# Emieeel/auto_oo

Hardware: NVIDIA B200
Metric: oo_energy_gradient_hessian_evals_per_sec (higher is better)
Workload: dtype f64

## Files before the change

auto_oo_b200/csrc/classes.cu:

```cuda
#include "common.cuh"

namespace oo {

int dgemm_tn(const double *At, const double *B, double *C, int64_t M, int64_t N, int64_t K,
             int64_t lda, int64_t ldb, int64_t ldc, int batch, int64_t strideA, int64_t strideB,
             int64_t strideC, cudaStream_t stream);
int dgemm_tn_swap02(const double *At, const double *B, double *C, double *C2, int d0, int d1, int d2,
                    int64_t N, int64_t K, int64_t lda, int64_t ldb, int64_t ldc, int batch, int64_t strideA,
                    int64_t strideB, int64_t strideC, cudaStream_t stream);
int dgemm_tn_pair_unpack(const double *At, const double *B, double *C, double *C2, int d0, int dorb, int dP,
                         int64_t N, int64_t K, int64_t lda, int64_t ldb, int64_t ldc, int batch,
                         int64_t strideA, int64_t strideB, int64_t strideC, int64_t strideC2,
                         cudaStream_t stream);

int dgemm_tn_class_pack(const double *At, const double *B, double *P, int tri_rows, int nclass, int dorb,
                        int64_t nrows2, int64_t npair_ld, int64_t K, int64_t lda, int64_t ldb, int batch,
                        int64_t strideA, int64_t strideB, int64_t strideP, cudaStream_t stream, int64_t r2_offset = 0);

int dgemm_tn_q1_packed8(const double *A8, int64_t a8_ld, int pq_lo, int pq_cnt, const double *B, double *C,
                        double *C2, int dorb, int dP, int64_t N, int64_t K, int64_t ldb, int64_t ldc, int batch,
                        int64_t strideA8, int64_t strideB, int64_t strideC, int64_t strideC2, cudaStream_t stream,
                        bool direct_epilogue);
bool dgemm_tn_tri_supported(int nclass);
int dgemm_tn_tri_class_pack(const double *At, const double *B, double *P, int tri_rows, int nclass, int dorb,
                            int64_t ngroups, int64_t npair_ld, int64_t K, int64_t lda, int64_t ldb, int batch,
                            int64_t strideA, int64_t strideB, int64_t strideP, cudaStream_t stream,
                            int64_t group_offset = 0, int64_t group_ld = 0, int halves = 1);

int dgemm_tn_class_expand(const double *At, const double *B, double *Out, int transpose_mirror, int nclass, int dorb,
                          int64_t npair_ld, int64_t K, int64_t lda, int64_t ldb, int64_t ld_out, int batch,
                          int64_t strideA, int64_t strideB, int64_t strideOut, cudaStream_t stream,
                          bool direct_epilogue = false);
int dgemm_tn_direct(const double *At, const double *B, double *C, int64_t M, int64_t N, int64_t K,
                    int64_t lda, int64_t ldb, int64_t ldc, int batch, int64_t strideA, int64_t strideB,
                    int64_t strideC, cudaStream_t stream);

namespace {

__global__ void __launch_bounds__(256) transpose_kernel(const double *__restrict__ src,
                                                        double *__restrict__ dst, int64_t rows,
                                                        int64_t cols) {
    __shared__ double tile[32][33];
    const int64_t c0 = (int64_t)blockIdx.x * 32, r0 = (int64_t)blockIdx.y * 32;
    const int tx = threadIdx.x & 31, ty = threadIdx.x >> 5;
#pragma unroll
    for (int j = ty; j < 32; j += 8) {
        const int64_t r = r0 + j, c = c0 + tx;
        if (r < rows && c < cols) tile[j][tx] = src[r * cols + c];
    }
    __syncthreads();
#pragma unroll
    for (int j = ty; j < 32; j += 8) {
        const int64_t c = c0 + j, r = r0 + tx;
        if (r < rows && c < cols) dst[c * rows + r] = tile[tx][j];
    }
}

}

int transpose(const double *src, double *dst, int64_t rows, int64_t cols, cudaStream_t stream) {
// ... 289 lines not shown
    if (!run(0)) {
    } else if (flags & OO_FLAG_CLASS_ERI_8FOLD) {
        if (slab) {
            OO_CUDA_CHECK(cudaMemsetAsync(T1t, 0, (size_t)batch * sT1t * sizeof(double), stream));
            OO_CUDA_CHECK(cudaMemsetAsync(P0, 0, (size_t)batch * sXp * sizeof(double), stream));
        }
        if (npairs) {
            concat_class_columns_kernel<<<dim3((unsigned)ld, (unsigned)npairs), 64, 0, stream>>>(C, strideC, ld, nIp, X);
            OO_LAUNCH_CHECK();
            if ((rc = dgemm_tn_q1_packed8(gpk, ldp, 0, (int)ldp, X, T1, T1t, ld, (int)ldp, 2 * nIp, ld, 2 * nIp, 2 * nIp,
                                          npairs, 0, (int64_t)ld * 2 * nIp, 2 * sT1, 2 * sT1t, stream, direct)))
                return rc;
        }
        if (nsingle &&
            (rc = dgemm_tn_q1_packed8(gpk + first_single * strideG, slab ? slab_ld : ldp, slab ? (int)pq_lo : 0,
                                      slab ? (int)pq_cnt : (int)ldp, C + first_single * strideC, T1 + first_single * sT1,
                                      T1t + first_single * sT1t, ld, (int)ldp, nIp, ld, ld, nIp, nsingle, strideG, strideC,
                                      sT1, sT1t, stream, direct)))
            return rc;
    } else if ((rc = dgemm_tn_pair_unpack(gpk, C, T1, T1t, ld, ld, (int)ldp, nIp, ld, (int64_t)ld * ldp, ld, nIp,
                                          batch, strideG, strideC, sT1, sT1t, stream))) {
        return rc;
    }
    if (!run(1)) {
    } else if (g_class_unfused_pack) {
        const dim3 pgrid((unsigned)ld2, (unsigned)batch);
        Q(T1, sT1, X, sX, ldp * nIp, nIp);
        pack_class_pairs_kernel<<<pgrid, 128, 0, stream>>>(X, P0, ld, nIp, (int)npIp, 1, sX, sXp);
        OO_LAUNCH_CHECK();
    } else if (tri_q2) {
        const int64_t g_lo = slab ? pq_lo : 0, g_cnt = slab ? pq_cnt : ldp;
        if (npairs &&
            (rc = dgemm_tn_tri_class_pack(T1, C, P0, 1, nIp, ld, ldp, npIp, ld, ldp * 2 * nIp, ld, npairs, 2 * sT1,
                                          strideC, sXp, stream, 0, 2 * nIp, 2)))
            return rc;
        if (nsingle &&
            (rc = dgemm_tn_tri_class_pack(T1 + first_single * sT1 + g_lo * nIp, C + first_single * strideC,
                                          P0 + first_single * sXp, 1, nIp, ld, g_cnt, npIp, ld, ldp * nIp, ld, nsingle,
                                          sT1, strideC, sXp, stream, g_lo)))
            return rc;
    } else {
        const int64_t g_lo = slab ? pq_lo : 0, g_cnt = slab ? pq_cnt : ldp;
        if ((rc = dgemm_tn_class_pack(T1 + g_lo * nIp, C, P0, 1, nIp, ld, g_cnt, npIp, ld, ldp * nIp, ld, batch, sT1,
                                      strideC, sXp, stream, g_lo)))
            return rc;
    }
    if (run(2)) Q(P0, sXp, P1, sXp, ld * npIp, ld);
    if (!run(3)) {
    } else if (g_class_unfused_pack) {
        Q(P1, sXp, Jp, sXp, npIp * ld, ld);
    } else if ((rc = dgemm_tn_class_expand(P1, C, Jout, 0, nIp, ld, npIp, ld, npIp * ld, ld, ld, batch, sXp,
                                           strideC, sCls, stream, direct))) {
        return rc;
    }
    if (!run(4)) {
    } else if (g_class_unfused_pack) {
        const dim3 pgrid((unsigned)ld2, (unsigned)batch);
        Q(T1t, sT1t, X, sX, ld2 * nIp, nIp);
        pack_class_pairs_kernel<<<pgrid, 128, 0, stream>>>(X, P0, ld, nIp, (int)npIp, 0, sX, sXp);
        OO_LAUNCH_CHECK();
    } else if (tri_q2) {
        if (npairs &&
            (rc = dgemm_tn_tri_class_pack(T1t, C, P0, 0, nIp, ld, ld2, npIp, ld, ld2 * 2 * nIp, ld, npairs, 2 * sT1t,
                                          strideC, sXp, stream, 0, 2 * nIp, 2)))
            return rc;
        if (nsingle &&
            (rc = dgemm_tn_tri_class_pack(T1t + first_single * sT1t, C + first_single * strideC, P0 + first_single * sXp,
                                          0, nIp, ld, ld2, npIp, ld, ld2 * nIp, ld, nsingle, sT1t, strideC, sXp, stream)))
            return rc;
    } else if ((rc = dgemm_tn_class_pack(T1t, C, P0, 0, nIp, ld, ld2, npIp, ld, ld2 * nIp, ld, batch, sT1t, strideC,
                                         sXp, stream))) {
        return rc;
    }
    if (run(5)) Q(P0, sXp, P1, sXp, ld * npIp, ld);
    if (!run(6)) return OO_OK;
    if (g_class_unfused_pack) {
        Q(P1, sXp, Kp, sXp, npIp * ld, ld);
    } else {
        if ((rc = dgemm_tn_class_expand(P1, C, Kout, 1, nIp, ld, npIp, ld, npIp * ld, ld, ld, batch, sXp, strideC,
                                        sCls, stream, direct)))
            return rc;
        return OO_OK;
    }
#undef Q
    const unsigned t = (unsigned)ceil_div(ld, 32);
    expand_class_kernel<<<dim3(t, t, (unsigned)(npI * batch)), 256, 0, stream>>>(Jp, Kp, cls, ld, nIp, (int)npI,
                                                                                 sXp, sCls);
    OO_LAUNCH_CHECK();
    return OO_OK;
}

}

extern "C" {

int oo_transpose_f64(const double *src, double *dst, int64_t rows, int64_t cols, void *stream) {
    return oo::transpose(src, dst, rows, cols, (cudaStream_t)stream);
}

int oo_eri_symmetry_defect_f64(const double *g_ao, int ld, double *defect3, void *stream) {
    return oo::eri_symmetry_defect(g_ao, ld, defect3, (cudaStream_t)stream);
// ... 34 lines not shown
```

auto_oo_b200/csrc/common.cuh:

```cuda
#pragma once

#include <cuda.h>
#include <cuda_runtime.h>
#include <stdint.h>
#include <stddef.h>

#include "../../include/oo_b200.h"

namespace oo {

extern int g_last_cuda_error;
extern unsigned long long g_launch_count;

inline int cuda_fail(cudaError_t e) {
    g_last_cuda_error = (int)e;
    return OO_ERR_CUDA;
}

#define OO_CUDA_CHECK(expr)                                   \
    do {                                                      \
        cudaError_t _e = (expr);                              \
        if (_e != cudaSuccess) return ::oo::cuda_fail(_e);    \
    } while (0)

// ... 10 lines not shown

inline int64_t ceil_div(int64_t a, int64_t b) { return (a + b - 1) / b; }
inline size_t align_up(size_t a, size_t b) { return (a + b - 1) / b * b; }

int sm_count();

inline bool once_per_device(unsigned long long &mask) {
    int dev = 0;
    if (cudaGetDevice(&dev) != cudaSuccess || dev < 0 || dev > 63) return true;
    const unsigned long long bit = 1ull << dev;
    if (mask & bit) return false;
    mask |= bit;
    return true;
}

__device__ __forceinline__ void dmma884(double &c0, double &c1, double a, double b) {
    asm volatile("mma.sync.aligned.m8n8k4.row.col.f64.f64.f64.f64 {%0,%1}, {%2}, {%3}, {%0,%1};"
                 : "+d"(c0), "+d"(c1)
                 : "d"(a), "d"(b));
}

__device__ __forceinline__ uint32_t smem_u32(const void *p) {
    return (uint32_t)__cvta_generic_to_shared(p);
}

__device__ __forceinline__ void mbar_init(uint64_t *bar, uint32_t count) {
    asm volatile("mbarrier.init.shared::cta.b64 [%0], %1;" ::"r"(smem_u32(bar)), "r"(count));
}

__device__ __forceinline__ void fence_barrier_init() {
    asm volatile("fence.mbarrier_init.release.cluster;" ::: "memory");
}

__device__ __forceinline__ void fence_proxy_async() {
    asm volatile("fence.proxy.async.shared::cta;" ::: "memory");
}

__device__ __forceinline__ void mbar_arrive_expect_tx(uint64_t *bar, uint32_t bytes) {
    asm volatile("mbarrier.arrive.expect_tx.shared::cta.b64 _, [%0], %1;" ::"r"(smem_u32(bar)),
                 "r"(bytes)
                 : "memory");
}

__device__ __forceinline__ void mbar_arrive(uint64_t *bar) {
    asm volatile("mbarrier.arrive.shared::cta.b64 _, [%0];" ::"r"(smem_u32(bar)) : "memory");
}

__device__ __forceinline__ void mbar_arrive_addr(uint32_t bar_smem_addr) {
    asm volatile("mbarrier.arrive.shared::cta.b64 _, [%0];" ::"r"(bar_smem_addr) : "memory");
}

__device__ __forceinline__ bool mbar_try_wait(uint64_t *bar, uint32_t parity) {
    uint32_t done;
    asm volatile(
        "{\n"
        ".reg .pred p;\n"
        "mbarrier.try_wait.parity.shared::cta.b64 p, [%1], %2;\n"
        "selp.u32 %0, 1, 0, p;\n"
        "}\n"
        : "=r"(done)
        : "r"(smem_u32(bar)), "r"(parity)
        : "memory");
    return done != 0;
}

__device__ __forceinline__ void mbar_wait(uint64_t *bar, uint32_t parity) {
// ... 75 lines not shown
```

auto_oo_b200/csrc/dgemm_tn.cu:

```cuda
#include "common.cuh"

namespace oo {

template <int BM_, int BN_, int BK_, int WGM_, int WGN_, int STAGES_, int NTC_ = 0>
struct TnCfg {
    static constexpr int BM = BM_, BN = BN_, BK = BK_, WGM = WGM_, WGN = WGN_, STAGES = STAGES_;
    static constexpr int NCW = WGM * WGN;
    static constexpr int THREADS = (NCW + 4) * 32;
    static_assert(NCW == 8, "register re-allocation below assumes 2 consumer warpgroups + 1 producer warpgroup");
    static constexpr int WTM = BM / WGM, WTN = BN / WGN;
    static constexpr int MT = WTM / 8, NT = NTC_ ? NTC_ : WTN / 8;
    static_assert(NTC_ == 0 || (WGN_ == 1 && NTC_ * 8 <= WTN), "a trimmed warp tile needs a single warp column");
    static constexpr int CHUNK_BYTES = BK * 128;
    static constexpr int A_BYTES = (BM / 16) * CHUNK_BYTES;
    static constexpr int B_BYTES = (BN / 16) * CHUNK_BYTES;
    static constexpr int STAGE_BYTES = A_BYTES + B_BYTES;
    static constexpr int SMEM_BYTES = STAGES * STAGE_BYTES + 2 * STAGES * 8 + 1024;
    static constexpr int LIN_PITCH = BM * 8 + 16;
    static constexpr int LIN_A_BYTES = (BK * LIN_PITCH + 1023) / 1024 * 1024;
    static constexpr int LIN_STAGE_BYTES = LIN_A_BYTES + B_BYTES;
    static constexpr int LIN_SMEM_BYTES = STAGES * LIN_STAGE_BYTES + 2 * STAGES * 8 + 1024;
    static constexpr int EPI_STAGES = 3;
    static constexpr int EPI_TILE_BYTES = BM * BN * 8;
    static constexpr int EPI_SMEM_BYTES = EPI_STAGES * LIN_STAGE_BYTES + EPI_TILE_BYTES + 2 * EPI_STAGES * 8 + 1024;
    static constexpr int EPI0_PITCH = BN * 8 + 16;
    static constexpr int EPI0_TILE_BYTES = BM * EPI0_PITCH;
    static constexpr int EPI0_STAGES = (227 * 1024 - 1024 - 64 - EPI0_TILE_BYTES) / STAGE_BYTES >= 4 ? 4
                                       : (227 * 1024 - 1024 - 64 - EPI0_TILE_BYTES) / STAGE_BYTES;
    static constexpr int EPI0_SMEM_BYTES = EPI0_STAGES * STAGE_BYTES + EPI0_TILE_BYTES + 2 * 4 * 8 + 1024;
    static_assert(WTM % 16 == 0 && WTN % 16 == 0, "warp tile must cover whole 16-wide chunks");
    static_assert(BK % 8 == 0, "BK must be a multiple of 8");
    static_assert((BK / 4) % 2 == 0, "the substep double buffer assumes an even number of substeps per k-block");
    static_assert(CHUNK_BYTES % 1024 == 0, "chunks must keep the 1024B swizzle alignment");
};

struct TnArgs {
    double *C;
    double *C2;
    int d0, d1, d2;
    int64_t M, N;
    int64_t ldc, strideC, strideC2;
    int kblocks;
    int tiles_m, tiles_n, batch;
    int a_batched, b_batched;
    const double *A8;
    int64_t strideA8;
    int K;
    int pq_lo, pq_cnt;
    int64_t a8_ld;
    int64_t r2_offset;
    int sym_T, sym_tiles_per_batch;
    int last_subs;
    uint32_t zero;
};

struct FalseTag { static constexpr bool value = false; };
struct TrueTag { static constexpr bool value = true; };

__device__ __forceinline__ void bulk_store_1d(void *gdst, uint32_t smem_src, uint32_t bytes) {
    asm volatile("cp.async.bulk.global.shared::cta.bulk_group [%0], [%1], %2;" ::"l"(gdst), "r"(smem_src), "r"(bytes)
                 : "memory");
}
__device__ __forceinline__ void named_bar_sync(int id, int nthreads) {
    asm volatile("bar.sync %0, %1;" ::"r"(id), "r"(nthreads) : "memory");
}
__device__ __forceinline__ void named_bar_arrive(int id, int nthreads) {
    asm volatile("bar.arrive %0, %1;" ::"r"(id), "r"(nthreads) : "memory");
}

__device__ __forceinline__ void bulk_load_1d(uint32_t smem_dst, const void *gsrc, uint32_t bytes, uint64_t *bar) {
    asm volatile("cp.async.bulk.shared::cluster.global.mbarrier::complete_tx::bytes [%0], [%1], %2, [%3];" ::"r"(smem_dst),
                 "l"(gsrc), "r"(bytes), "r"(smem_u32(bar))
                 : "memory");
}

template <class Cfg, int DUAL, int AMODE = 0, int EPI = 0>
__global__ void __launch_bounds__(Cfg::THREADS, 1)
dgemm_tn_kernel(const __grid_constant__ CUtensorMap mapA, const __grid_constant__ CUtensorMap mapB,
                const TnArgs args) {
    static_assert(EPI == 0 || (DUAL == 2 && AMODE == 1) || (AMODE == 0 && (DUAL == 0 || DUAL == 5)),
                  "the staged epilogue exists for quarter 1 and for the plain / class-expand stores");
    constexpr int STAGE_BYTES = AMODE ? Cfg::LIN_STAGE_BYTES : Cfg::STAGE_BYTES;
    constexpr int A_BYTES = AMODE ? Cfg::LIN_A_BYTES : Cfg::A_BYTES;
    constexpr int NST = !EPI ? Cfg::STAGES : (AMODE ? Cfg::EPI_STAGES : (Cfg::EPI0_STAGES > 0 ? Cfg::EPI0_STAGES : 1));
    constexpr int kShipWarps = 3;
    constexpr int kBarFree = 1, kBarFull = 2, kBarThreads = (Cfg::NCW + kShipWarps) * 32;
    constexpr int TILE_BYTES = AMODE ? Cfg::EPI_TILE_BYTES : Cfg::EPI0_TILE_BYTES;
    extern __shared__ uint8_t smem_raw[];
    const uint32_t smem_base = (smem_u32(smem_raw) + 1023u) & ~1023u;
    uint8_t *smem = smem_raw + (smem_base - smem_u32(smem_raw));
    const uint32_t ctile = smem_base + NST * STAGE_BYTES;
    uint64_t *full_bar = reinterpret_cast<uint64_t *>(smem + NST * STAGE_BYTES + (EPI ? TILE_BYTES : 0));
    uint64_t *empty_bar = full_bar + NST;

    const int warp = threadIdx.x >> 5;
    const int lane = threadIdx.x & 31;

    if (threadIdx.x == 0) {
#pragma unroll
        for (int s = 0; s < NST; ++s) {
            mbar_init(&full_bar[s], 1);
// ... 767 lines not shown
```

auto_oo_b200/csrc/dgemm_tri.cu:

```cuda
#include "common.cuh"

namespace oo {

int encode_tmap_4d_f64(CUtensorMap *map, const void *base, const uint64_t dims[4], const uint64_t strides_elems[3],
                       const uint32_t box[4]);

namespace {

template <int GP_, int MTC_, int STAGES_>
struct TriCfg {
    static constexpr int GP = GP_, STAGES = STAGES_, BK = 16;
    static constexpr int NCW = 8;
    static constexpr int THREADS = (NCW + 4) * 32;
    static constexpr int MT = MTC_;
    static_assert(MTC_ * 8 <= GP_, "class tiles exceed the group");
    static constexpr int CPG = GP / 16;
    static constexpr int CHUNK_BYTES = BK * 128;
    static constexpr int A_BYTES = NCW * CPG * CHUNK_BYTES;
    static constexpr int B_BYTES = CPG * CHUNK_BYTES;
    static constexpr int STAGE_BYTES = A_BYTES + B_BYTES;
    static constexpr int SMEM_BYTES = STAGES * STAGE_BYTES + 2 * STAGES * 8 + 1024;
    static_assert((STAGES & (STAGES - 1)) == 0, "STAGES must be a power of two");
    static_assert(SMEM_BYTES <= 227 * 1024, "stage ring exceeds the shared memory of an SM");
};

struct TriArgs {
    double *P;
    int64_t npair_ld, strideP;
    int nclass;
    int tri_rows;
    int dorb;
    int64_t ngroups;
    int64_t group_offset;
    int kblocks, tiles_per_batch, batch;
    int halves;
    int a_batched, b_batched;
    int last_subs;
    uint32_t zero;
};

struct FalseTag { static constexpr bool value = false; };
struct TrueTag { static constexpr bool value = true; };

__device__ __forceinline__ void tma_load_4d(void *smem_dst, const CUtensorMap *map, uint64_t *bar, int c0, int c1,
                                            int c2, int c3) {
    asm volatile(
        "cp.async.bulk.tensor.4d.shared::cluster.global.mbarrier::complete_tx::bytes"
        " [%0], [%1, {%3, %4, %5, %6}], [%2];" ::"r"(smem_u32(smem_dst)),
        "l"(map), "r"(smem_u32(bar)), "r"(c0), "r"(c1), "r"(c2), "r"(c3)
        : "memory");
}

template <class Cfg>
__global__ void __launch_bounds__(Cfg::THREADS, 1)
dgemm_tn_tri_kernel(const __grid_constant__ CUtensorMap mapA, const __grid_constant__ CUtensorMap mapB,
                    const TriArgs args) {
    extern __shared__ uint8_t smem_raw[];
    const uint32_t smem_base = (smem_u32(smem_raw) + 1023u) & ~1023u;
    uint8_t *smem = smem_raw + (smem_base - smem_u32(smem_raw));
    uint64_t *full_bar = reinterpret_cast<uint64_t *>(smem + Cfg::STAGES * Cfg::STAGE_BYTES);
    uint64_t *empty_bar = full_bar + Cfg::STAGES;
    const int warp = threadIdx.x >> 5, lane = threadIdx.x & 31;

    if (threadIdx.x == 0) {
#pragma unroll
        for (int s = 0; s < Cfg::STAGES; ++s) {
            mbar_init(&full_bar[s], 1);
            mbar_init(&empty_bar[s], Cfg::NCW);
        }
        fence_barrier_init();
        tma_prefetch_desc(&mapA);
        tma_prefetch_desc(&mapB);
    }
    __syncthreads();
    const int64_t total_tiles = (int64_t)args.tiles_per_batch * args.batch;

    if (warp >= Cfg::NCW) {
        asm volatile("setmaxnreg.dec.sync.aligned.u32 40;");
        if (warp == Cfg::NCW && lane == 0) {
            int stage = 0;
            uint32_t phase = 0;
            for (int64_t tile = blockIdx.x; tile < total_tiles; tile += gridDim.x) {
                const int b = (int)(tile / args.tiles_per_batch);
                const int u = (int)(tile - (int64_t)b * args.tiles_per_batch);
                const int h = u % args.halves, g0 = (u / args.halves) * Cfg::NCW;
                const int ba = args.a_batched ? b : 0, bb = args.b_batched ? b * args.halves + h : 0;
                const int m0 = h * args.nclass;
                for (int kb = 0; kb < args.kblocks; ++kb) {
                    mbar_wait(&empty_bar[stage], phase ^ 1u);
                    mbar_arrive_expect_tx(&full_bar[stage], Cfg::STAGE_BYTES);
                    uint8_t *sA = smem + stage * Cfg::STAGE_BYTES;
                    uint8_t *sB = sA + Cfg::A_BYTES;
                    const int k0 = kb * Cfg::BK;
#pragma unroll
                    for (int w = 0; w < Cfg::NCW; ++w)
#pragma unroll
                        for (int c = 0; c < Cfg::CPG; ++c)
                            tma_load_4d(sA + (w * Cfg::CPG + c) * Cfg::CHUNK_BYTES, &mapA, &full_bar[stage],
                                        m0 + 16 * c, g0 + w, k0, ba);
#pragma unroll
                    for (int c = 0; c < Cfg::CPG; ++c)
                        tma_load_3d(sB + c * Cfg::CHUNK_BYTES, &mapB, &full_bar[stage], 16 * c, k0, bb);
                    if (++stage == Cfg::STAGES) {
                        stage = 0;
                        phase ^= 1u;
                    }
                }
            }
        }
        return;
    }
    asm volatile("setmaxnreg.inc.sync.aligned.u32 232;");
    const int g = lane >> 2, t = lane & 3;
    uint32_t x[2][2];
#pragma unroll
    for (int h = 0; h < 2; ++h)
#pragma unroll
        for (int j = 0; j < 2; ++j) {
            const uint32_t krow = 2 * t + j;
            x[h][j] = krow * 128u + ((((uint32_t)(h * 8 + g)) * 8u) ^ (krow << 4));
        }
    const uint32_t a_warp_off = (uint32_t)(warp * Cfg::CPG) * Cfg::CHUNK_BYTES;
    constexpr int MT = Cfg::MT;
    constexpr int SUB = Cfg::BK / 4;

    uint32_t it = 0;
    for (uint32_t tile = blockIdx.x; tile < (uint32_t)total_tiles; tile += gridDim.x) {
        double acc[MT][MT][2];
#pragma unroll
        for (int mi = 0; mi < MT; ++mi)
#pragma unroll
            for (int ni = 0; ni <= mi; ++ni) acc[mi][ni][0] = acc[mi][ni][1] = 0.0;
        double a[2][MT], bf[2][MT];
        uint32_t loaded = 0, loaded_next = 0;
        auto load_frags = [&](int buf, uint32_t st, int sub, uint32_t &lx) {
            const uint32_t sbase = smem_base + st * Cfg::STAGE_BYTES;
            const uint32_t abase = sbase + a_warp_off, bbase = sbase + Cfg::A_BYTES;
            const int kk = sub >> 1, j = sub & 1;
#pragma unroll
            for (int mi = 0; mi < MT; ++mi)
                a[buf][mi] = lds_f64(abase + (mi >> 1) * Cfg::CHUNK_BYTES + kk * 1024 + x[mi & 1][j]);
#pragma unroll
            for (int ni = 0; ni < MT; ++ni)
                bf[buf][ni] = lds_f64(bbase + (ni >> 1) * Cfg::CHUNK_BYTES + kk * 1024 + x[ni & 1][j]);
#pragma unroll
            for (int mi = 0; mi < MT; ++mi) lx ^= (uint32_t)__double2hiint(a[buf][mi]);
#pragma unroll
            for (int ni = 0; ni < MT; ++ni) lx ^= (uint32_t)__double2hiint(bf[buf][ni]);
        };
        {
            const uint32_t stage = it & (Cfg::STAGES - 1);
            mbar_wait(&full_bar[stage], (it / Cfg::STAGES) & 1u);
            load_frags(0, stage, 0, loaded);
        }
        auto kblock = [&](auto last_tag) {
            constexpr bool LAST = decltype(last_tag)::value;
            const uint32_t stage = it & (Cfg::STAGES - 1);
#pragma unroll
            for (int sub = 0; sub < SUB; ++sub) {
                const int cur = sub & 1, nxt = cur ^ 1;
                if (sub + 1 < SUB) {
                    load_frags(nxt, stage, sub + 1, loaded);
                } else if (!LAST) {
                    const uint32_t nstage = (it + 1) & (Cfg::STAGES - 1);
                    mbar_wait(&full_bar[nstage], ((it + 1) / Cfg::STAGES) & 1u);
                    load_frags(nxt, nstage, 0, loaded_next);
                }
                if (!LAST || sub < args.last_subs) {
#pragma unroll
                    for (int mi = 0; mi < MT; ++mi)
#pragma unroll
                        for (int ni = 0; ni <= mi; ++ni)
                            dmma884(acc[mi][ni][0], acc[mi][ni][1], a[cur][mi], bf[cur][ni]);
                }
            }
            if (lane == 0) mbar_arrive_addr(smem_u32(&empty_bar[stage]) + (loaded & args.zero));
            loaded = loaded_next;
            loaded_next = 0;
            ++it;
        };
        for (int kb = 0; kb + 1 < args.kblocks; ++kb) kblock(FalseTag{});
        kblock(TrueTag{});

        const int b = (int)(tile / (uint32_t)args.tiles_per_batch);
        const int u = (int)(tile - (uint32_t)b * (uint32_t)args.tiles_per_batch);
        const int64_t grp = (int64_t)(u / args.halves) * Cfg::NCW + warp;
        if (grp >= args.ngroups) continue;
        double *row0 = nullptr, *row1 = nullptr;
        double *base = args.P + (int64_t)(b * args.halves + u % args.halves) * args.strideP;
        if (args.tri_rows) {
            const int64_t pq = grp + args.group_offset;
            int p = (int)((sqrt(8.0 * (double)pq + 1.0) - 1.0) * 0.5);
            while ((int64_t)(p + 1) * (p + 2) / 2 <= pq) ++p;
            while ((int64_t)p * (p + 1) / 2 > pq) --p;
            const int q = (int)(pq - (int64_t)p * (p + 1) / 2);
            if (p >= args.dorb) continue;
            row0 = base + ((int64_t)p * args.dorb + q) * args.npair_ld;
            row1 = base + ((int64_t)q * args.dorb + p) * args.npair_ld;
        } else {
            row0 = row1 = base + grp * args.npair_ld;
        }
#pragma unroll
        for (int mi = 0; mi < MT; ++mi) {
            const int m = mi * 8 + g;
            if (m >= args.nclass) continue;
            const int64_t off = (int64_t)m * (m + 1) / 2;
#pragma unroll
            for (int ni = 0; ni <= mi; ++ni)
#pragma unroll
                for (int c = 0; c < 2; ++c) {
                    const int n = ni * 8 + 2 * t + c;
                    if (n <= m) {
                        row0[off + n] = acc[mi][ni][c];
                        if (row1 != row0) row1[off + n] = acc[mi][ni][c];
                    }
                }
        }
    }
}

template <class Cfg>
int launch_tri(const double *At, const double *B, double *P, int tri_rows, int nclass, int dorb, int64_t ngroups,
               int64_t npair_ld, int64_t K, int64_t lda, int64_t ldb, int batch, int64_t strideA, int64_t strideB,
               int64_t strideP, cudaStream_t stream, int64_t group_offset, int64_t group_ld, int halves) {
    CUtensorMap mapA, mapB;
    const int a_batched = (batch > 1 && strideA != 0);
    const int b_batched = ((batch > 1 || halves > 1) && strideB != 0);
    const uint64_t dimsA[4] = {(uint64_t)(halves > 1 ? group_ld : nclass), (uint64_t)ngroups, (uint64_t)K,
                               (uint64_t)(a_batched ? batch : 1)};
    const uint64_t strA[3] = {(uint64_t)group_ld, (uint64_t)lda, (uint64_t)(a_batched ? strideA : lda * K)};
    const uint32_t boxA[4] = {16, 1, (uint32_t)Cfg::BK, 1};
    int rc = encode_tmap_4d_f64(&mapA, At, dimsA, strA, boxA);
    if (rc) return rc;
    rc = encode_tmap_3d_f64(&mapB, B, (uint64_t)nclass, (uint64_t)K, b_batched ? batch * halves : 1, (uint64_t)ldb,
                            b_batched ? (uint64_t)strideB : (uint64_t)ldb * K, 16, Cfg::BK);
    if (rc) return rc;
    TriArgs args;
    args.P = P;
    args.npair_ld = npair_ld;
    args.strideP = strideP;
    args.nclass = nclass;
    args.tri_rows = tri_rows;
    args.dorb = dorb;
    args.ngroups = ngroups;
    args.group_offset = group_offset;
    args.kblocks = (int)ceil_div(K, Cfg::BK);
    args.tiles_per_batch = (int)ceil_div(ngroups, Cfg::NCW) * halves;
    args.batch = batch;
    args.halves = halves;
    args.a_batched = a_batched;
    args.b_batched = b_batched;
    args.last_subs = 2 * (int)ceil_div(K - (int64_t)(args.kblocks - 1) * Cfg::BK, 8);
    args.zero = 0;
    static unsigned long long attr_set = 0;
    if (once_per_device(attr_set))
        OO_CUDA_CHECK(cudaFuncSetAttribute(dgemm_tn_tri_kernel<Cfg>, cudaFuncAttributeMaxDynamicSharedMemorySize,
                                           Cfg::SMEM_BYTES));
    const int64_t total = (int64_t)args.tiles_per_batch * batch;
    const int grid = (int)(total < sm_count() ? total : sm_count());
    dgemm_tn_tri_kernel<Cfg><<<grid, Cfg::THREADS, Cfg::SMEM_BYTES, stream>>>(mapA, mapB, args);
    OO_LAUNCH_CHECK();
    return OO_OK;
}

}

bool dgemm_tn_tri_supported(int nclass) { return nclass > 16 && nclass <= 48 && (nclass % 2) == 0; }

int dgemm_tn_tri_class_pack(const double *At, const double *B, double *P, int tri_rows, int nclass, int dorb,
                            int64_t ngroups, int64_t npair_ld, int64_t K, int64_t lda, int64_t ldb, int batch,
                            int64_t strideA, int64_t strideB, int64_t strideP, cudaStream_t stream,
                            int64_t group_offset, int64_t group_ld, int halves) {
    OO_REQUIRE(At && B && P && nclass > 0 && ngroups > 0 && K > 0 && batch > 0 && dorb > 0);
    if (group_ld == 0) group_ld = nclass;
    OO_REQUIRE((halves == 1 || halves == 2) && group_ld >= (int64_t)halves * nclass && (group_ld % 2) == 0);
    OO_REQUIRE(lda >= (ngroups - 1) * group_ld + (int64_t)halves * nclass);
    OO_REQUIRE(dgemm_tn_tri_supported(nclass) && npair_ld >= (int64_t)nclass * (nclass + 1) / 2);
    OO_REQUIRE((lda % 2) == 0 && (ldb % 2) == 0 && (strideA % 2) == 0 && (strideB % 2) == 0);
    OO_REQUIRE(((uintptr_t)At % 16) == 0 && ((uintptr_t)B % 16) == 0);
    if (ngroups * halves >= (1ll << 31) || K >= (1ll << 31)) return OO_ERR_UNSUPPORTED;
#define OO_TRI(GP, MTC)                                                                                              \
    return launch_tri<TriCfg<GP, MTC, 4>>(At, B, P, tri_rows, nclass, dorb, ngroups, npair_ld, K, lda, ldb, batch, strideA, \
                                          strideB, strideP, stream, group_offset, group_ld, halves)
    if (nclass <= 24) OO_TRI(32, 3);
    if (nclass <= 32) OO_TRI(32, 4);
    if (nclass <= 40) OO_TRI(48, 5);
    OO_TRI(48, 6);
#undef OO_TRI
}

}
```

Measured before the change: 77.31.

## Stage tri-pack epilogue through shared memory with bulk stores and fold partial atoms

The triangular class-pack kernel gains a staged epilogue: consumer warps write packed lower-triangle results into a per-warp shared slot, and dedicated ship warps copy them to global memory with bulk async stores, synchronised through named barriers. This is meant to overlap the output stores with the next tile's MMA work. A fold mode spreads the last partial 8-row atom across warp pairs to skip wasted MMAs when nclass mod 8 is small. The A tensor-map layout changes to load all 8 warp groups in one box, BK drops to 8, and register budgets are rebalanced with setmaxnreg. The cost is extra shared memory, more barrier traffic, and more complex code paths.

```diff
diff --git a/auto_oo_b200/csrc/classes.cu b/auto_oo_b200/csrc/classes.cu
--- a/auto_oo_b200/csrc/classes.cu
+++ b/auto_oo_b200/csrc/classes.cu
@@ -25,7 +25,8 @@
 int dgemm_tn_tri_class_pack(const double *At, const double *B, double *P, int tri_rows, int nclass, int dorb,
                             int64_t ngroups, int64_t npair_ld, int64_t K, int64_t lda, int64_t ldb, int batch,
                             int64_t strideA, int64_t strideB, int64_t strideP, cudaStream_t stream,
-                            int64_t group_offset = 0, int64_t group_ld = 0, int halves = 1);
+                            int64_t group_offset = 0, int64_t group_ld = 0, int halves = 1,
+                            bool direct_epilogue = false);
 
 int dgemm_tn_class_expand(const double *At, const double *B, double *Out, int transpose_mirror, int nclass, int dorb,
                           int64_t npair_ld, int64_t K, int64_t lda, int64_t ldb, int64_t ld_out, int batch,
@@ -381,12 +382,12 @@
         const int64_t g_lo = slab ? pq_lo : 0, g_cnt = slab ? pq_cnt : ldp;
         if (npairs &&
             (rc = dgemm_tn_tri_class_pack(T1, C, P0, 1, nIp, ld, ldp, npIp, ld, ldp * 2 * nIp, ld, npairs, 2 * sT1,
-                                          strideC, sXp, stream, 0, 2 * nIp, 2)))
+                                          strideC, sXp, stream, 0, 2 * nIp, 2, direct)))
             return rc;
         if (nsingle &&
             (rc = dgemm_tn_tri_class_pack(T1 + first_single * sT1 + g_lo * nIp, C + first_single * strideC,
                                           P0 + first_single * sXp, 1, nIp, ld, g_cnt, npIp, ld, ldp * nIp, ld, nsingle,
-                                          sT1, strideC, sXp, stream, g_lo)))
+                                          sT1, strideC, sXp, stream, g_lo, 0, 1, direct)))
             return rc;
     } else {
         const int64_t g_lo = slab ? pq_lo : 0, g_cnt = slab ? pq_cnt : ldp;
@@ -411,11 +412,12 @@
     } else if (tri_q2) {
         if (npairs &&
             (rc = dgemm_tn_tri_class_pack(T1t, C, P0, 0, nIp, ld, ld2, npIp, ld, ld2 * 2 * nIp, ld, npairs, 2 * sT1t,
-                                          strideC, sXp, stream, 0, 2 * nIp, 2)))
+                                          strideC, sXp, stream, 0, 2 * nIp, 2, direct)))
             return rc;
         if (nsingle &&
             (rc = dgemm_tn_tri_class_pack(T1t + first_single * sT1t, C + first_single * strideC, P0 + first_single * sXp,
-                                          0, nIp, ld, ld2, npIp, ld, ld2 * nIp, ld, nsingle, sT1t, strideC, sXp, stream)))
+                                          0, nIp, ld, ld2, npIp, ld, ld2 * nIp, ld, nsingle, sT1t, strideC, sXp, stream,
+                                          0, 0, 1, direct)))
             return rc;
     } else if ((rc = dgemm_tn_class_pack(T1t, C, P0, 0, nIp, ld, ld2, npIp, ld, ld2 * nIp, ld, batch, sT1t, strideC,
                                          sXp, stream))) {
diff --git a/auto_oo_b200/csrc/common.cuh b/auto_oo_b200/csrc/common.cuh
--- a/auto_oo_b200/csrc/common.cuh
+++ b/auto_oo_b200/csrc/common.cuh
@@ -66,6 +66,16 @@
     asm volatile("fence.mbarrier_init.release.cluster;" ::: "memory");
 }
 
+__device__ __forceinline__ void bulk_store_1d(void *gdst, uint32_t smem_src, uint32_t bytes) {
+    asm volatile("cp.async.bulk.global.shared::cta.bulk_group [%0], [%1], %2;" ::"l"(gdst), "r"(smem_src), "r"(bytes)
+                 : "memory");
+}
+__device__ __forceinline__ void named_bar_sync(int id, int nthreads) {
+    asm volatile("bar.sync %0, %1;" ::"r"(id), "r"(nthreads) : "memory");
+}
+__device__ __forceinline__ void named_bar_arrive(int id, int nthreads) {
+    asm volatile("bar.arrive %0, %1;" ::"r"(id), "r"(nthreads) : "memory");
+}
 __device__ __forceinline__ void fence_proxy_async() {
     asm volatile("fence.proxy.async.shared::cta;" ::: "memory");
 }
diff --git a/auto_oo_b200/csrc/dgemm_tn.cu b/auto_oo_b200/csrc/dgemm_tn.cu
--- a/auto_oo_b200/csrc/dgemm_tn.cu
+++ b/auto_oo_b200/csrc/dgemm_tn.cu
@@ -56,17 +56,6 @@
 
 struct FalseTag { static constexpr bool value = false; };
 struct TrueTag { static constexpr bool value = true; };
-
-__device__ __forceinline__ void bulk_store_1d(void *gdst, uint32_t smem_src, uint32_t bytes) {
-    asm volatile("cp.async.bulk.global.shared::cta.bulk_group [%0], [%1], %2;" ::"l"(gdst), "r"(smem_src), "r"(bytes)
-                 : "memory");
-}
-__device__ __forceinline__ void named_bar_sync(int id, int nthreads) {
-    asm volatile("bar.sync %0, %1;" ::"r"(id), "r"(nthreads) : "memory");
-}
-__device__ __forceinline__ void named_bar_arrive(int id, int nthreads) {
-    asm volatile("bar.arrive %0, %1;" ::"r"(id), "r"(nthreads) : "memory");
-}
 
 __device__ __forceinline__ void bulk_load_1d(uint32_t smem_dst, const void *gsrc, uint32_t bytes, uint64_t *bar) {
     asm volatile("cp.async.bulk.shared::cluster.global.mbarrier::complete_tx::bytes [%0], [%1], %2, [%3];" ::"r"(smem_dst),
diff --git a/auto_oo_b200/csrc/dgemm_tri.cu b/auto_oo_b200/csrc/dgemm_tri.cu
--- a/auto_oo_b200/csrc/dgemm_tri.cu
+++ b/auto_oo_b200/csrc/dgemm_tri.cu
@@ -9,7 +9,7 @@
 
 template <int GP_, int MTC_, int STAGES_>
 struct TriCfg {
-    static constexpr int GP = GP_, STAGES = STAGES_, BK = 16;
+    static constexpr int GP = GP_, STAGES = STAGES_, BK = 8;
     static constexpr int NCW = 8;
     static constexpr int THREADS = (NCW + 4) * 32;
     static constexpr int MT = MTC_;
@@ -19,7 +19,9 @@
     static constexpr int A_BYTES = NCW * CPG * CHUNK_BYTES;
     static constexpr int B_BYTES = CPG * CHUNK_BYTES;
     static constexpr int STAGE_BYTES = A_BYTES + B_BYTES;
-    static constexpr int SMEM_BYTES = STAGES * STAGE_BYTES + 2 * STAGES * 8 + 1024;
+    static constexpr int TRI_SLOT_BYTES = (GP * (GP + 1) / 2 + 1) / 2 * 16;
+    static constexpr int EPI_TILE_BYTES = NCW * TRI_SLOT_BYTES;
+    static constexpr int SMEM_BYTES = STAGES * STAGE_BYTES + EPI_TILE_BYTES + 2 * STAGES * 8 + 1024;
     static_assert((STAGES & (STAGES - 1)) == 0, "STAGES must be a power of two");
     static_assert(SMEM_BYTES <= 227 * 1024, "stage ring exceeds the shared memory of an SM");
 };
@@ -36,8 +38,34 @@
     int halves;
     int a_batched, b_batched;
     int last_subs;
+    int fold;
+    int staged;
     uint32_t zero;
 };
+
+constexpr int kTriShipWarps = 3, kTriBarFree = 1, kTriBarFull = 2, kTriBarThreads = (8 + kTriShipWarps) * 32;
+
+__device__ __forceinline__ void sts_f64(uint32_t addr, double v) {
+    asm volatile("st.shared.f64 [%0], %1;" ::"r"(addr), "d"(v) : "memory");
+}
+
+__device__ __forceinline__ bool tri_group_rows(const TriArgs &args, double *base, int64_t grp, double *&row0,
+                                               double *&row1) {
+    if (grp >= args.ngroups) return false;
+    if (args.tri_rows) {
+        const int64_t pq = grp + args.group_offset;
+        int p = (int)((sqrt(8.0 * (double)pq + 1.0) - 1.0) * 0.5);
+        while ((int64_t)(p + 1) * (p + 2) / 2 <= pq) ++p;
+        while ((int64_t)p * (p + 1) / 2 > pq) --p;
+        const int q = (int)(pq - (int64_t)p * (p + 1) / 2);
+        if (p >= args.dorb) return false;
+        row0 = base + ((int64_t)p * args.dorb + q) * args.npair_ld;
+        row1 = base + ((int64_t)q * args.dorb + p) * args.npair_ld;
+    } else {
+        row0 = row1 = base + grp * args.npair_ld;
+    }
+    return true;
+}
 
 struct FalseTag { static constexpr bool value = false; };
 struct TrueTag { static constexpr bool value = true; };
@@ -51,6 +79,191 @@
         : "memory");
 }
 
+template <class Cfg, bool FOLD>
+__device__ __forceinline__ void tri_consumer(const uint32_t smem_base, uint64_t *full_bar, uint64_t *empty_bar,
+                                             const TriArgs &args, const int warp, const int lane,
+                                             const int64_t total_tiles) {
+    constexpr int MT = Cfg::MT;
+    constexpr int OWN = FOLD ? MT - 1 : MT;
+    constexpr int NF = FOLD ? (MT + 1) / 2 : 0;
+    constexpr int NFA = NF > 0 ? NF : 1;
+    static_assert(!FOLD || 2 * NF * 8 <= Cfg::GP, "the shared atom's column atoms exceed the B tile");
+    constexpr int SUB = Cfg::BK / 4;
+    const int g = lane >> 2, t = lane & 3;
+    uint32_t x[2][2];
+#pragma unroll
+    for (int h = 0; h < 2; ++h)
+#pragma unroll
+        for (int j = 0; j < 2; ++j) {
+            const uint32_t krow = 2 * t + j;
+            x[h][j] = krow * 128u + ((((uint32_t)(h * 8 + g)) * 8u) ^ (krow << 4));
+        }
+    const uint32_t a_warp_off = (uint32_t)warp * Cfg::CHUNK_BYTES;
+    const int fold_row = 8 * (MT - 1) + (g & 3), fold_warp = (warp & ~1) | (g >> 2), fold_col = (warp & 1) * NF;
+    uint32_t fa[2], fb[NFA][2];
+#pragma unroll
+    for (int j = 0; j < 2; ++j) {
+        const uint32_t krow = 2 * t + j;
+        fa[j] = (uint32_t)((fold_row >> 4) * Cfg::NCW + fold_warp) * Cfg::CHUNK_BYTES + krow * 128u +
+                ((((uint32_t)(fold_row & 15)) * 8u) ^ (krow << 4));
+#pragma unroll
+        for (int f = 0; f < NFA; ++f) {
+            const int n8 = fold_col + f;
+            fb[f][j] = Cfg::A_BYTES + (uint32_t)(n8 >> 1) * Cfg::CHUNK_BYTES + krow * 128u +
+                       ((((uint32_t)((n8 & 1) * 8 + g)) * 8u) ^ (krow << 4));
+        }
+    }
+
+    uint32_t it = 0;
+    for (uint32_t tile = blockIdx.x; tile < (uint32_t)total_tiles; tile += gridDim.x) {
+        double acc[OWN][OWN][2], accf[NFA][2];
+#pragma unroll
+        for (int mi = 0; mi < OWN; ++mi)
+#pragma unroll
+            for (int ni = 0; ni <= mi; ++ni) acc[mi][ni][0] = acc[mi][ni][1] = 0.0;
+#pragma unroll
+        for (int f = 0; f < NFA; ++f) accf[f][0] = accf[f][1] = 0.0;
+        double a[2][OWN], bf[2][OWN], af[2], bff[2][NFA];
+        uint32_t loaded = 0, loaded_next = 0;
+        auto load_frags = [&](int buf, uint32_t st, int sub, uint32_t &lx) {
+            const uint32_t sbase = smem_base + st * Cfg::STAGE_BYTES;
+            const uint32_t abase = sbase + a_warp_off, bbase = sbase + Cfg::A_BYTES;
+            const int kk = sub >> 1, j = sub & 1;
+#pragma unroll
+            for (int mi = 0; mi < OWN; ++mi)
+                a[buf][mi] = lds_f64(abase + (mi >> 1) * Cfg::NCW * Cfg::CHUNK_BYTES + kk * 1024 + x[mi & 1][j]);
+#pragma unroll
+            for (int ni = 0; ni < OWN; ++ni)
+                bf[buf][ni] = lds_f64(bbase + (ni >> 1) * Cfg::CHUNK_BYTES + kk * 1024 + x[ni & 1][j]);
+#pragma unroll
+            for (int mi = 0; mi < OWN; ++mi) lx ^= (uint32_t)__double2hiint(a[buf][mi]);
+#pragma unroll
+            for (int ni = 0; ni < OWN; ++ni) lx ^= (uint32_t)__double2hiint(bf[buf][ni]);
+            if (FOLD) {
+                af[buf] = lds_f64(sbase + fa[j] + kk * 1024);
+                lx ^= (uint32_t)__double2hiint(af[buf]);
+#pragma unroll
+                for (int f = 0; f < NF; ++f) {
+                    bff[buf][f] = lds_f64(sbase + fb[f][j] + kk * 1024);
+                    lx ^= (uint32_t)__double2hiint(bff[buf][f]);
+                }
+            }
+        };
+        {
+            const uint32_t stage = it & (Cfg::STAGES - 1);
+            mbar_wait(&full_bar[stage], (it / Cfg::STAGES) & 1u);
+            load_frags(0, stage, 0, loaded);
+        }
+        auto kblock = [&](auto last_tag) {
+            constexpr bool LAST = decltype(last_tag)::value;
+            const uint32_t stage = it & (Cfg::STAGES - 1);
+#pragma unroll
+            for (int sub = 0; sub < SUB; ++sub) {
+                const int cur = sub & 1, nxt = cur ^ 1;
+                if (sub + 1 < SUB) {
+                    load_frags(nxt, stage, sub + 1, loaded);
+                } else if (!LAST) {
+                    const uint32_t nstage = (it + 1) & (Cfg::STAGES - 1);
+                    mbar_wait(&full_bar[nstage], ((it + 1) / Cfg::STAGES) & 1u);
+                    load_frags(nxt, nstage, 0, loaded_next);
+                }
+                if (!LAST || sub < args.last_subs) {
+#pragma unroll
+                    for (int mi = 0; mi < OWN; ++mi)
+#pragma unroll
+                        for (int ni = 0; ni <= mi; ++ni)
+                            dmma884(acc[mi][ni][0], acc[mi][ni][1], a[cur][mi], bf[cur][ni]);
+                    if (FOLD) {
+#pragma unroll
+                        for (int f = 0; f < NF; ++f) dmma884(accf[f][0], accf[f][1], af[cur], bff[cur][f]);
+                    }
+                }
+            }
+            if (lane == 0) mbar_arrive_addr(smem_u32(&empty_bar[stage]) + (loaded & args.zero));
+            loaded = loaded_next;
+            loaded_next = 0;
+            ++it;
+        };
+        for (int kb = 0; kb + 1 < args.kblocks; ++kb) kblock(FalseTag{});
+        kblock(TrueTag{});
+
+        if (args.staged) {
+            const uint32_t slot = smem_base + Cfg::STAGES * Cfg::STAGE_BYTES + (uint32_t)warp * Cfg::TRI_SLOT_BYTES;
+            named_bar_sync(kTriBarFree, kTriBarThreads);
+#pragma unroll
+            for (int mi = 0; mi < OWN; ++mi) {
+                const int m = mi * 8 + g;
+                if (m >= args.nclass) continue;
+                const uint32_t off = (uint32_t)(m * (m + 1) / 2);
+#pragma unroll
+                for (int ni = 0; ni <= mi; ++ni)
+#pragma unroll
+                    for (int c = 0; c < 2; ++c) {
+                        const int n = ni * 8 + 2 * t + c;
+                        if (n <= m) sts_f64(slot + (off + n) * 8u, acc[mi][ni][c]);
+                    }
+            }
+            if (FOLD && fold_row < args.nclass) {
+                const int m = fold_row;
+                const uint32_t fslot = slot + (uint32_t)(fold_warp - warp) * Cfg::TRI_SLOT_BYTES;
+                const uint32_t off = (uint32_t)(m * (m + 1) / 2);
+#pragma unroll
+                for (int f = 0; f < NF; ++f)
+#pragma unroll
+                    for (int c = 0; c < 2; ++c) {
+                        const int n = (fold_col + f) * 8 + 2 * t + c;
+                        if (n <= m) sts_f64(fslot + (off + n) * 8u, accf[f][c]);
+                    }
+            }
+            const int ntri = args.nclass * (args.nclass + 1) / 2;
+            if ((ntri & 1) && lane == 0) sts_f64(slot + (uint32_t)ntri * 8u, 0.0);
+            fence_proxy_async();
+            named_bar_arrive(kTriBarFull, kTriBarThreads);
+            continue;
+        }
+        const int b = (int)(tile / (uint32_t)args.tiles_per_batch);
+        const int u = (int)(tile - (uint32_t)b * (uint32_t)args.tiles_per_batch);
+        const int64_t g0 = (int64_t)(u / args.halves) * Cfg::NCW;
+        double *base = args.P + (int64_t)(b * args.halves + u % args.halves) * args.strideP;
+        auto group_rows = [&](int64_t grp, double *&row0, double *&row1) {
+            return tri_group_rows(args, base, grp, row0, row1);
+        };
+        double *row0 = nullptr, *row1 = nullptr;
+        if (group_rows(g0 + warp, row0, row1)) {
+#pragma unroll
+            for (int mi = 0; mi < OWN; ++mi) {
+                const int m = mi * 8 + g;
+                if (m >= args.nclass) continue;
+                const int64_t off = (int64_t)m * (m + 1) / 2;
+#pragma unroll
+                for (int ni = 0; ni <= mi; ++ni)
+#pragma unroll
+                    for (int c = 0; c < 2; ++c) {
+                        const int n = ni * 8 + 2 * t + c;
+                        if (n <= m) {
+                            row0[off + n] = acc[mi][ni][c];
+                            if (row1 != row0) row1[off + n] = acc[mi][ni][c];
+                        }
+                    }
+            }
+        }
+        if (FOLD && fold_row < args.nclass && group_rows(g0 + fold_warp, row0, row1)) {
+            const int m = fold_row;
+            const int64_t off = (int64_t)m * (m + 1) / 2;
+#pragma unroll
+            for (int f = 0; f < NF; ++f)
+#pragma unroll
+                for (int c = 0; c < 2; ++c) {
+                    const int n = (fold_col + f) * 8 + 2 * t + c;
+                    if (n <= m) {
+                        row0[off + n] = accf[f][c];
+                        if (row1 != row0) row1[off + n] = accf[f][c];
+                    }
+                }
+        }
+    }
+}
+
 template <class Cfg>
 __global__ void __launch_bounds__(Cfg::THREADS, 1)
 dgemm_tn_tri_kernel(const __grid_constant__ CUtensorMap mapA, const __grid_constant__ CUtensorMap mapB,
@@ -58,7 +271,8 @@
     extern __shared__ uint8_t smem_raw[];
     const uint32_t smem_base = (smem_u32(smem_raw) + 1023u) & ~1023u;
     uint8_t *smem = smem_raw + (smem_base - smem_u32(smem_raw));
-    uint64_t *full_bar = reinterpret_cast<uint64_t *>(smem + Cfg::STAGES * Cfg::STAGE_BYTES);
+    const uint32_t etile = smem_base + Cfg::STAGES * Cfg::STAGE_BYTES;
+    uint64_t *full_bar = reinterpret_cast<uint64_t *>(smem + Cfg::STAGES * Cfg::STAGE_BYTES + Cfg::EPI_TILE_BYTES);
     uint64_t *empty_bar = full_bar + Cfg::STAGES;
     const int warp = threadIdx.x >> 5, lane = threadIdx.x & 31;
 
@@ -76,7 +290,7 @@
     const int64_t total_tiles = (int64_t)args.tiles_per_batch * args.batch;
 
     if (warp >= Cfg::NCW) {
-        asm volatile("setmaxnreg.dec.sync.aligned.u32 40;");
+        asm volatile("setmaxnreg.dec.sync.aligned.u32 64;");
         if (warp == Cfg::NCW && lane == 0) {
             int stage = 0;
             uint32_t phase = 0;
@@ -93,11 +307,9 @@
                     uint8_t *sB = sA + Cfg::A_BYTES;
                     const int k0 = kb * Cfg::BK;
 #pragma unroll
-                    for (int w = 0; w < Cfg::NCW; ++w)
-#pragma unroll
-                        for (int c = 0; c < Cfg::CPG; ++c)
-                            tma_load_4d(sA + (w * Cfg::CPG + c) * Cfg::CHUNK_BYTES, &mapA, &full_bar[stage],
-                                        m0 + 16 * c, g0 + w, k0, ba);
+                    for (int c = 0; c < Cfg::CPG; ++c)
+                        tma_load_4d(sA + c * Cfg::NCW * Cfg::CHUNK_BYTES, &mapA, &full_bar[stage], m0 + 16 * c, k0,
+                                    g0, ba);
 #pragma unroll
                     for (int c = 0; c < Cfg::CPG; ++c)
                         tma_load_3d(sB + c * Cfg::CHUNK_BYTES, &mapB, &full_bar[stage], 16 * c, k0, bb);
@@ -107,129 +319,52 @@
                     }
                 }
             }
+        } else if (args.staged && warp > Cfg::NCW) {
+            const int sw = warp - Cfg::NCW - 1;
+            const uint32_t bytes = (uint32_t)((args.nclass * (args.nclass + 1) / 2 + 1) / 2) * 16u;
+            named_bar_arrive(kTriBarFree, kTriBarThreads);
+            for (int64_t tile = blockIdx.x; tile < total_tiles; tile += gridDim.x) {
+                const int b = (int)(tile / args.tiles_per_batch);
+                const int u = (int)(tile - (int64_t)b * args.tiles_per_batch);
+                const int64_t g0 = (int64_t)(u / args.halves) * Cfg::NCW;
+                double *base = args.P + (int64_t)(b * args.halves + u % args.halves) * args.strideP;
+                named_bar_sync(kTriBarFull, kTriBarThreads);
+                if (lane < Cfg::NCW && lane % kTriShipWarps == sw) {
+                    double *row0, *row1;
+                    if (tri_group_rows(args, base, g0 + lane, row0, row1)) {
+                        const uint32_t src = etile + (uint32_t)lane * Cfg::TRI_SLOT_BYTES;
+                        bulk_store_1d(row0, src, bytes);
+                        if (row1 != row0) bulk_store_1d(row1, src, bytes);
+                    }
+                }
+                asm volatile("cp.async.bulk.commit_group;" ::: "memory");
+                asm volatile("cp.async.bulk.wait_group.read 0;" ::: "memory");
+                __syncwarp();
+                named_bar_arrive(kTriBarFree, kTriBarThreads);
+            }
+            asm volatile("cp.async.bulk.wait_group 0;" ::: "memory");
         }
         return;
     }
-    asm volatile("setmaxnreg.inc.sync.aligned.u32 232;");
-    const int g = lane >> 2, t = lane & 3;
-    uint32_t x[2][2];
-#pragma unroll
-    for (int h = 0; h < 2; ++h)
-#pragma unroll
-        for (int j = 0; j < 2; ++j) {
-            const uint32_t krow = 2 * t + j;
-            x[h][j] = krow * 128u + ((((uint32_t)(h * 8 + g)) * 8u) ^ (krow << 4));
-        }
-    const uint32_t a_warp_off = (uint32_t)(warp * Cfg::CPG) * Cfg::CHUNK_BYTES;
-    constexpr int MT = Cfg::MT;
-    constexpr int SUB = Cfg::BK / 4;
-
-    uint32_t it = 0;
-    for (uint32_t tile = blockIdx.x; tile < (uint32_t)total_tiles; tile += gridDim.x) {
-        double acc[MT][MT][2];
-#pragma unroll
-        for (int mi = 0; mi < MT; ++mi)
-#pragma unroll
-            for (int ni = 0; ni <= mi; ++ni) acc[mi][ni][0] = acc[mi][ni][1] = 0.0;
-        double a[2][MT], bf[2][MT];
-        uint32_t loaded = 0, loaded_next = 0;
-        auto load_frags = [&](int buf, uint32_t st, int sub, uint32_t &lx) {
-            const uint32_t sbase = smem_base + st * Cfg::STAGE_BYTES;
-            const uint32_t abase = sbase + a_warp_off, bbase = sbase + Cfg::A_BYTES;
-            const int kk = sub >> 1, j = sub & 1;
-#pragma unroll
-            for (int mi = 0; mi < MT; ++mi)
-                a[buf][mi] = lds_f64(abase + (mi >> 1) * Cfg::CHUNK_BYTES + kk * 1024 + x[mi & 1][j]);
-#pragma unroll
-            for (int ni = 0; ni < MT; ++ni)
-                bf[buf][ni] = lds_f64(bbase + (ni >> 1) * Cfg::CHUNK_BYTES + kk * 1024 + x[ni & 1][j]);
-#pragma unroll
-            for (int mi = 0; mi < MT; ++mi) lx ^= (uint32_t)__double2hiint(a[buf][mi]);
-#pragma unroll
-            for (int ni = 0; ni < MT; ++ni) lx ^= (uint32_t)__double2hiint(bf[buf][ni]);
-        };
-        {
-            const uint32_t stage = it & (Cfg::STAGES - 1);
-            mbar_wait(&full_bar[stage], (it / Cfg::STAGES) & 1u);
-            load_frags(0, stage, 0, loaded);
-        }
-        auto kblock = [&](auto last_tag) {
-            constexpr bool LAST = decltype(last_tag)::value;
-            const uint32_t stage = it & (Cfg::STAGES - 1);
-#pragma unroll
-            for (int sub = 0; sub < SUB; ++sub) {
-                const int cur = sub & 1, nxt = cur ^ 1;
-                if (sub + 1 < SUB) {
-                    load_frags(nxt, stage, sub + 1, loaded);
-                } else if (!LAST) {
-                    const uint32_t nstage = (it + 1) & (Cfg::STAGES - 1);
-                    mbar_wait(&full_bar[nstage], ((it + 1) / Cfg::STAGES) & 1u);
-                    load_frags(nxt, nstage, 0, loaded_next);
-                }
-                if (!LAST || sub < args.last_subs) {
-#pragma unroll
-                    for (int mi = 0; mi < MT; ++mi)
-#pragma unroll
-                        for (int ni = 0; ni <= mi; ++ni)
-                            dmma884(acc[mi][ni][0], acc[mi][ni][1], a[cur][mi], bf[cur][ni]);
-                }
-            }
-            if (lane == 0) mbar_arrive_addr(smem_u32(&empty_bar[stage]) + (loaded & args.zero));
-            loaded = loaded_next;
-            loaded_next = 0;
-            ++it;
-        };
-        for (int kb = 0; kb + 1 < args.kblocks; ++kb) kblock(FalseTag{});
-        kblock(TrueTag{});
-
-        const int b = (int)(tile / (uint32_t)args.tiles_per_batch);
-        const int u = (int)(tile - (uint32_t)b * (uint32_t)args.tiles_per_batch);
-        const int64_t grp = (int64_t)(u / args.halves) * Cfg::NCW + warp;
-        if (grp >= args.ngroups) continue;
-        double *row0 = nullptr, *row1 = nullptr;
-        double *base = args.P + (int64_t)(b * args.halves + u % args.halves) * args.strideP;
-        if (args.tri_rows) {
-            const int64_t pq = grp + args.group_offset;
-            int p = (int)((sqrt(8.0 * (double)pq + 1.0) - 1.0) * 0.5);
-            while ((int64_t)(p + 1) * (p + 2) / 2 <= pq) ++p;
-            while ((int64_t)p * (p + 1) / 2 > pq) --p;
-            const int q = (int)(pq - (int64_t)p * (p + 1) / 2);
-            if (p >= args.dorb) continue;
-            row0 = base + ((int64_t)p * args.dorb + q) * args.npair_ld;
-            row1 = base + ((int64_t)q * args.dorb + p) * args.npair_ld;
-        } else {
-            row0 = row1 = base + grp * args.npair_ld;
-        }
-#pragma unroll
-        for (int mi = 0; mi < MT; ++mi) {
-            const int m = mi * 8 + g;
-            if (m >= args.nclass) continue;
-            const int64_t off = (int64_t)m * (m + 1) / 2;
-#pragma unroll
-            for (int ni = 0; ni <= mi; ++ni)
-#pragma unroll
-                for (int c = 0; c < 2; ++c) {
-                    const int n = ni * 8 + 2 * t + c;
-                    if (n <= m) {
-                        row0[off + n] = acc[mi][ni][c];
-                        if (row1 != row0) row1[off + n] = acc[mi][ni][c];
-                    }
-                }
-        }
-    }
+    static_assert(128 * (168 - 64) >= 256 * (216 - 168), "setmaxnreg.inc would wait for registers never released");
+    asm volatile("setmaxnreg.inc.sync.aligned.u32 216;");
+    if (args.fold) tri_consumer<Cfg, true>(smem_base, full_bar, empty_bar, args, warp, lane, total_tiles);
+    else tri_consumer<Cfg, false>(smem_base, full_bar, empty_bar, args, warp, lane, total_tiles);
 }
 
 template <class Cfg>
 int launch_tri(const double *At, const double *B, double *P, int tri_rows, int nclass, int dorb, int64_t ngroups,
                int64_t npair_ld, int64_t K, int64_t lda, int64_t ldb, int batch, int64_t strideA, int64_t strideB,
-               int64_t strideP, cudaStream_t stream, int64_t group_offset, int64_t group_ld, int halves) {
+               int64_t strideP, cudaStream_t stream, int64_t group_offset, int64_t group_ld, int halves,
+               bool direct_epilogue) {
+    OO_REQUIRE(ceil_div(nclass, 8) == Cfg::MT);
     CUtensorMap mapA, mapB;
     const int a_batched = (batch > 1 && strideA != 0);
     const int b_batched = ((batch > 1 || halves > 1) && strideB != 0);
-    const uint64_t dimsA[4] = {(uint64_t)(halves > 1 ? group_ld : nclass), (uint64_t)ngroups, (uint64_t)K,
+    const uint64_t dimsA[4] = {(uint64_t)(halves > 1 ? group_ld : nclass), (uint64_t)K, (uint64_t)ngroups,
                                (uint64_t)(a_batched ? batch : 1)};
-    const uint64_t strA[3] = {(uint64_t)group_ld, (uint64_t)lda, (uint64_t)(a_batched ? strideA : lda * K)};
-    const uint32_t boxA[4] = {16, 1, (uint32_t)Cfg::BK, 1};
+    const uint64_t strA[3] = {(uint64_t)lda, (uint64_t)group_ld, (uint64_t)(a_batched ? strideA : lda * K)};
+    const uint32_t boxA[4] = {16, (uint32_t)Cfg::BK, (uint32_t)Cfg::NCW, 1};
     int rc = encode_tmap_4d_f64(&mapA, At, dimsA, strA, boxA);
     if (rc) return rc;
     rc = encode_tmap_3d_f64(&mapB, B, (uint64_t)nclass, (uint64_t)K, b_batched ? batch * halves : 1, (uint64_t)ldb,
@@ -251,6 +386,10 @@
     args.a_batched = a_batched;
     args.b_batched = b_batched;
     args.last_subs = 2 * (int)ceil_div(K - (int64_t)(args.kblocks - 1) * Cfg::BK, 8);
+    args.fold = (nclass % 8) != 0 && (nclass % 8) <= 4;
+    const int64_t ntri16 = ((int64_t)nclass * (nclass + 1) / 2 + 1) / 2 * 2;
+    args.staged = !direct_epilogue && npair_ld >= ntri16 && (npair_ld % 2) == 0 && (strideP % 2) == 0 &&
+                  ((uintptr_t)P % 16) == 0;
     args.zero = 0;
     static unsigned long long attr_set = 0;
     if (once_per_device(attr_set))
@@ -270,7 +409,7 @@
 int dgemm_tn_tri_class_pack(const double *At, const double *B, double *P, int tri_rows, int nclass, int dorb,
                             int64_t ngroups, int64_t npair_ld, int64_t K, int64_t lda, int64_t ldb, int batch,
                             int64_t strideA, int64_t strideB, int64_t strideP, cudaStream_t stream,
-                            int64_t group_offset, int64_t group_ld, int halves) {
+                            int64_t group_offset, int64_t group_ld, int halves, bool direct_epilogue) {
     OO_REQUIRE(At && B && P && nclass > 0 && ngroups > 0 && K > 0 && batch > 0 && dorb > 0);
     if (group_ld == 0) group_ld = nclass;
     OO_REQUIRE((halves == 1 || halves == 2) && group_ld >= (int64_t)halves * nclass && (group_ld % 2) == 0);
@@ -281,7 +420,8 @@
     if (ngroups * halves >= (1ll << 31) || K >= (1ll << 31)) return OO_ERR_UNSUPPORTED;
 #define OO_TRI(GP, MTC)                                                                                              \
     return launch_tri<TriCfg<GP, MTC, 4>>(At, B, P, tri_rows, nclass, dorb, ngroups, npair_ld, K, lda, ldb, batch, strideA, \
-                                          strideB, strideP, stream, group_offset, group_ld, halves)
+                                          strideB, strideP, stream, group_offset, group_ld, halves, \
+                                          direct_epilogue)
     if (nclass <= 24) OO_TRI(32, 3);
     if (nclass <= 32) OO_TRI(32, 4);
     if (nclass <= 40) OO_TRI(48, 5);
```

Result: faster. 79.40 (median of 6 runs) (+2.7%).
